# muellan/metacache

Measured on AMD Instinct MI355X. Metric: Mreads/min (150 bp), higher is better.
Workload: dtype u32

## Files before the change

metacache_amd/csrc/gw_kernels.hip:

```cpp
#include "device_common.h"

#include <algorithm>
#include <cstdlib>

namespace mcamd {

namespace {

constexpr uint32_t kGwNone = 0xFFFFFFFFu;
constexpr uint32_t kGwRounds = 128;
constexpr uint32_t kGwLoads = kGwRounds / 16;

struct __attribute__((packed, aligned(4))) U4 { uint32_t x, y, z, w; };

__device__ __forceinline__ uint32_t gw_block_shift(uint32_t maxWin)
{
    const uint32_t D = maxWin > 1 ? maxWin - 1 : 1;
    const uint32_t A = 32u - (uint32_t)__builtin_clz(64u * D - 1u);
    return A < 8u ? 8u : A;
}

template <uint32_t T1LOG2, uint32_t T2LOG2>
struct GwBloom {
    static constexpr uint32_t kW1 = (1u << T1LOG2) / 32, kW2 = (1u << T2LOG2) / 32, kWords = kW1 + kW2;
// ... 572 lines not shown
__device__ __forceinline__ uint32_t gw_count_numbers(const uint32_t (&v)[PER], uint2* slots, uint32_t* ck, const uint32_t lane)
{
    constexpr uint32_t kByteMask = ((1u << LOG2S) - 1u) << 3;
    char* base = reinterpret_cast<char*>(slots);
    auto key_at = [&](uint32_t off) -> uint32_t* { return reinterpret_cast<uint32_t*>(base + off); };
    uint32_t off[PER], old[PER];
    bool coll = false;
#pragma unroll
    for (uint32_t r = 0; r < PER; ++r) {
        off[r] = gw_slot<LOG2S>(v[r]);
        old[r] = v[r] != kGwNone ? atomicCAS(key_at(off[r]), kGwNone, v[r]) : v[r];
        coll = coll || (old[r] != kGwNone && old[r] != v[r]);
    }
    if (__ballot(coll)) {
#pragma unroll
        for (uint32_t r = 0; r < PER; ++r) {
            if (old[r] != kGwNone && old[r] != v[r]) {
                uint32_t o = off[r];
                for (;;) {
                    o = (o + 8u) & kByteMask;
                    old[r] = atomicCAS(key_at(o), kGwNone, v[r]);
                    if (old[r] == kGwNone || old[r] == v[r]) break;
                }
                off[r] = o;
            }
        }
    }
    uint32_t C = 0;
#pragma unroll
    for (uint32_t r = 0; r < PER; ++r) {
        if (v[r] != kGwNone) atomicAdd(key_at(off[r]) + 1, 1u);
        const bool claimed = v[r] != kGwNone && old[r] == kGwNone;
        const uint64_t m = __ballot(claimed);
        if (claimed) {
            const uint32_t at = __builtin_amdgcn_mbcnt_hi((uint32_t)(m >> 32), __builtin_amdgcn_mbcnt_lo((uint32_t)m, C));
            if (CKCAP == 0xFFFFFFFFu || at < CKCAP) ck[at] = off[r];
        }
        C += (uint32_t)__popcll(m);
    }
    return C;
}

template <uint32_t LOG2S, uint32_t PER, bool TAX>
__device__ __forceinline__ uint32_t gw_pick(const uint32_t* ck, const uint32_t C, uint2* slots, const uint32_t lane, const uint32_t maxWin,
                                            const uint32_t K, const uint32_t* __restrict__ taxkey, const DeviceTable& tab,
                                            uint32_t& owv, uint32_t& owh, uint32_t& owd)
{
    constexpr uint32_t kByteMask = ((1u << LOG2S) - 1u) << 3;
    const char* base = reinterpret_cast<const char*>(slots);
    uint32_t v[PER], R[PER];
#pragma unroll
    for (uint32_t r = 0; r < PER; ++r) {
        const uint2 c = r * 64 + lane < C ? *reinterpret_cast<const uint2*>(base + ck[r * 64 + lane]) : make_uint2(kGwNone, 0u);
        v[r] = c.x; R[r] = c.y;
    }
    uint32_t tgt[TAX ? PER : 1], thi[TAX ? PER : 1];
    if constexpr (TAX) {
#pragma unroll
        for (uint32_t r = 0; r < PER; ++r) tgt[r] = v[r] != kGwNone ? tab.gwDir[v[r] >> tab.gwDirShift] : 0u;
    }
    for (uint32_t d = 1; d < maxWin; ++d) {
        uint2 kc[PER]; uint32_t o[PER];
        bool chain = false;
#pragma unroll
        for (uint32_t r = 0; r < PER; ++r) {
            o[r] = gw_slot<LOG2S>(v[r] - d);
            kc[r] = *reinterpret_cast<const uint2*>(base + o[r]);
            if (v[r] == kGwNone) kc[r].x = kGwNone;
            chain = chain || (kc[r].x != v[r] - d && kc[r].x != kGwNone);
        }
        if (__ballot(chain)) {
#pragma unroll
            for (uint32_t r = 0; r < PER; ++r)
                while (kc[r].x != v[r] - d && kc[r].x != kGwNone) { o[r] = (o[r] + 8u) & kByteMask; kc[r] = *reinterpret_cast<const uint2*>(base + o[r]); }
        }
#pragma unroll
        for (uint32_t r = 0; r < PER; ++r)
            if (kc[r].x == v[r] - d) R[r] = ((R[r] & 0xFFFFu) + kc[r].y) | (d << 16);
    }
    uint32_t ptax[TAX ? PER : 1];
    if constexpr (TAX) {
#pragma unroll
        for (uint32_t r = 0; r < PER; ++r) {
            thi[r] = v[r] != kGwNone ? tab.gwBase[tgt[r] + 1] : 0u;
            while (v[r] != kGwNone && v[r] >= thi[r]) { ++tgt[r]; thi[r] = tab.gwBase[tgt[r] + 1]; }
            ptax[r] = v[r] != kGwNone ? taxkey[tgt[r]] : 0u;
        }
    }
    uint32_t live = 0;
#pragma unroll
    for (uint32_t r = 0; r < PER; ++r) {
        bool ok = v[r] != kGwNone;
        if constexpr (TAX) ok = ok && ptax[r] != 0;
        live |= ok ? (1u << r) : 0u;
    }
    uint32_t strong = 0;
    uint32_t wv = kGwNone, wh = 0, wd = 0;
    for (uint32_t rnd = 0; rnd < K; ++rnd) {
        uint32_t hh = 0, hv = kGwNone, hd = 0, hg = 0;
#pragma unroll
        for (uint32_t r = 0; r < PER; ++r) {
            const uint32_t h = R[r] & 0xFFFFu;
            const bool take = ((live >> r) & 1u) && (h > hh || (h == hh && v[r] < hv));
            if (take) { hh = h; hv = v[r]; hd = R[r] >> 16; if constexpr (TAX) hg = ptax[r]; }
        }
        const uint32_t mh = wave_max_u32(hh);
        if (mh == 0) break;
        const uint32_t mv = wave_min_u32(hh == mh ? hv : kGwNone);
        const uint32_t winner = __ffsll((unsigned long long)__ballot(hh == mh && hv == mv)) - 1;
        const uint32_t d = rdlane(hd, winner);
        if constexpr (TAX) {
            const uint32_t g = rdlane(hg, winner);
#pragma unroll
            for (uint32_t r = 0; r < PER; ++r) if (ptax[r] == g) live &= ~(1u << r);
        } else {
            const uint32_t from = mv - tab.gwGap, span = 2u * tab.gwGap;
#pragma unroll
            for (uint32_t r = 0; r < PER; ++r) if (v[r] - from <= span) live &= ~(1u << r);
        }
        if (lane == rnd) { wv = mv; wh = mh; wd = d; }
        strong += mh >= 2 ? 1u : 0u;
    }
    owv = wv; owh = wh; owd = wd;
    return strong;
}

template <bool TAX>
__device__ __forceinline__ bool gw_winners_out(const uint32_t lane, const uint32_t K, const uint32_t wv, const uint32_t wh, const uint32_t wd,
                                               const uint32_t wt, const uint32_t wlo, const uint32_t whi, mc_candidate_dev* __restrict__ out,
                                               uint32_t (&pickLo)[kLaneK], uint32_t (&pickHi)[kLaneK])
{
    bool again = false;
    if constexpr (!TAX) {
#pragma unroll
        for (uint32_t i = 0; i + 1 < kLaneK; ++i) {
            const uint32_t ti = rdlane(wt, i);
            again = again || (__ballot(lane > i && lane < K && wt == ti && ti != 0xFFFFFFFFu) != 0);
        }
    }
#pragma unroll
    for (uint32_t i = 0; i < kLaneK; ++i) { pickLo[i] = rdlane(wlo, i); pickHi[i] = rdlane(whi, i); }
    if (lane < K) {
        mc_candidate_dev e; e.tgt = wt; e.hits = wh; e.end = wv - wlo; e.beg = e.end - wd;
        if (wv == kGwNone) { e.tgt = 0xFFFFFFFFu; e.hits = 0; e.beg = 0; e.end = 0; }
        out[lane] = e;
    }
    return again;
}

}

namespace {

struct GwPend {
    bool pend = false;
    uint32_t q = 0, wv = kGwNone, wh = 0, wd = 0, dir = 0, b0 = 0, b1 = 0, b2 = 0;
    __device__ __forceinline__ void bases(const DeviceTable& tab)
    {
        if (pend && wv != kGwNone) { b0 = tab.gwBase[dir]; b1 = tab.gwBase[dir + 1]; b2 = tab.gwBase[min(dir + 2, tab.gwTargets)]; }
    }
    template <bool TAX>
    __device__ __forceinline__ void finish(const uint32_t lane, const uint32_t K, const DeviceTable& tab, const Workspace& ws, mc_candidate_dev* __restrict__ cands)
    {
        if (!pend) return;
        uint32_t t = 0xFFFFFFFFu, lo = 0, hi = 0;
        if (wv != kGwNone) {
            t = dir; lo = b0; hi = b1;
            if (wv >= b1) { ++t; lo = b1; hi = b2; }
            while (wv >= hi) { ++t; lo = hi; hi = tab.gwBase[t + 1]; }
        }
        uint32_t plo[kLaneK], phi[kLaneK];
        const bool again = gw_winners_out<TAX>(lane, K, wv, wh, wd, t, lo, hi, cands + (size_t)q * K, plo, phi);
        if (lane == 0) {
            if (again) { ws.hitScan[q] = ws.qstat[q].hits; ws.qflag[q] = kFlagCands; }
            else ws.qflag[q] = kFlagDone;
        }
        pend = false;
    }
};

template <uint32_t LOG2S, bool TAX, bool DEFER, bool LONG = false, class GetV, class EntF>
__device__ __forceinline__ bool gw_count_read(const uint32_t q, EntF&& entf, const uint32_t n2, const uint32_t maxWin, GetV&& getv,
                                              uint2* slots, uint32_t* ck, uint64_t* T, const uint32_t lane, const uint32_t grp, const uint32_t sub4,
                                              const uint32_t K, const uint32_t* __restrict__ taxkey, const DeviceTable& tab, const Workspace& ws,
                                              mc_candidate_dev* __restrict__ cands, GwPend& P)
{
    constexpr uint32_t kSlots = 1u << LOG2S, kList = kSlots / 2;
    {
        uint4* k4 = reinterpret_cast<uint4*>(slots);
#pragma unroll
        for (uint32_t i = 0; i < kSlots * 8 / 16 / 64; ++i) k4[i * 64 + lane] = make_uint4(kGwNone, 0u, kGwNone, 0u);
    }
    wave_lds_sync();
    uint32_t pickLo[kLaneK], pickHi[kLaneK];
#pragma unroll
    for (uint32_t i = 0; i < kLaneK; ++i) { pickLo[i] = 0; pickHi[i] = 0; }
    uint32_t strong = 0, wv = kGwNone, wh = 0, wd = 0;
    bool again = false;
    mc_candidate_dev* out = cands + (size_t)q * K;
    if constexpr (DEFER) P.bases(tab);
    uint32_t C = 0;
    auto body = [&](auto perc) {
        constexpr uint32_t PER = decltype(perc)::value;
        uint32_t v[PER];
#pragma unroll
        for (uint32_t r = 0; r < PER; ++r) v[r] = getv(r);
        C = gw_count_numbers<LOG2S, PER, LONG ? kList : 0xFFFFFFFFu>(v, slots, ck, lane);
    };
    const uint32_t per = (n2 + 63u) / 64u;
    if constexpr (LOG2S == 9) {
        if (per <= 1) body(std::integral_constant<uint32_t, 1>{});
        else if (per <= 2) body(std::integral_constant<uint32_t, 2>{});
        else if (per <= 3) body(std::integral_constant<uint32_t, 3>{});
        else if (!LONG || per <= 4) body(std::integral_constant<uint32_t, 4>{});
        else if constexpr (LONG) {
            if (per <= 6) body(std::integral_constant<uint32_t, 6>{});
            else body(std::integral_constant<uint32_t, 8>{});
        }
    } else if constexpr (LOG2S == 10) {
        if (per <= 6) body(std::integral_constant<uint32_t, 6>{});
        else body(std::integral_constant<uint32_t, 8>{});
    } else {
        if (per <= 10) body(std::integral_constant<uint32_t, 10>{});
        else if (per <= 12) body(std::integral_constant<uint32_t, 12>{});
        else body(std::integral_constant<uint32_t, kList / 64>{});
    }
    C = __builtin_amdgcn_readfirstlane(C);
    wave_lds_sync();
    if constexpr (LONG) {
        if (C > kList) {
            if constexpr (DEFER) P.template finish<TAX>(lane, K, tab, ws, cands);
            wave_lds_sync();
            return false;
        }
    }
    auto pick = [&](auto perc) {
        constexpr uint32_t PER = decltype(perc)::value;
        strong = gw_pick<LOG2S, PER, TAX>(ck, C, slots, lane, maxWin, K, taxkey, tab, wv, wh, wd);
    };
    if (C <= 64) pick(std::integral_constant<uint32_t, 1>{});
    else if (C <= 128) pick(std::integral_constant<uint32_t, 2>{});
    else if (C <= 256) pick(std::integral_constant<uint32_t, 4>{});
    else if constexpr (LOG2S >= 10) {
        if (C <= 512) pick(std::integral_constant<uint32_t, 8>{});
        else if constexpr (LOG2S >= 11) pick(std::integral_constant<uint32_t, 16>{});
    }
    strong = __builtin_amdgcn_readfirstlane(strong);
    if constexpr (DEFER) {
        P.template finish<TAX>(lane, K, tab, ws, cands);
        if (strong >= K) {
            P.pend = true; P.q = q; P.wv = wv; P.wh = wh; P.wd = wd;
            P.dir = wv != kGwNone ? tab.gwDir[wv >> tab.gwDirShift] : 0u;
            wave_lds_sync();
            return true;
        }
    }
    {
        uint32_t wt = 0xFFFFFFFFu, wlo = 0, whi = 0;
        if (wv != kGwNone) tab.gw_target_bounds(wv, wt, wlo, whi);
        again = gw_winners_out<TAX>(lane, K, wv, wh, wd, wt, wlo, whi, out, pickLo, pickHi);
    }
    bool done = true;
    if (again) {
        if (lane == 0) { ws.hitScan[q] = ws.qstat[q].hits; ws.qflag[q] = kFlagCands; }
        done = false;
    } else if (strong < K) {
        const uint2 r6 = entf();
        const uint32_t fbase = r6.x, nent = r6.y;
        if (TAX || nent > kBigEnt) {
            if (lane == 0) { ws.hitScan[q] = ws.qstat[q].hits; ws.qflag[q] = kFlagCands; }
            done = false;
        } else if constexpr (!TAX) {
            wave_lds_sync();
            const uint32_t sz = lane < nent ? (ws.psize[fbase + lane] & 0xFFFFu) : 0u;
            const uint64_t pay = lane < nent ? ws.ppay[fbase + lane] : 0ull;
            const uint32_t myR = sz > 1 ? (sz + 15u) >> 4 : 0u;
            const uint32_t incl = wave_incl_scan_u32(myR, lane), Rc = rdlane(incl, 63), start = incl - myR;
            uint32_t best[kLaneK];
#pragma unroll
            for (uint32_t i = 0; i < kLaneK; ++i) best[i] = kGwNone;
            uint32_t seen = 0;
            auto visit = [&](uint32_t g, bool valid) {
                if (!valid) return;
                bool skip = false;
#pragma unroll
                for (uint32_t i = 0; i < kLaneK; ++i) skip = skip || (i < strong && g - pickLo[i] < pickHi[i] - pickLo[i]);
                if (skip) return;
                ++seen;
                uint32_t c = g;
#pragma unroll
                for (uint32_t i = 0; i < kLaneK; ++i) { const uint32_t lo = min(best[i], c); c = max(best[i], c); best[i] = lo; }
            };
            visit(sz == 1 ? tab.gw_of(pay) : kGwNone, sz == 1);
            for (uint32_t r0 = 0; r0 < Rc; r0 += kGwRounds) {
                for (uint32_t i = lane; i < kGwRounds; i += 64) if (r0 + i >= Rc) T[i] = 0ull;
                const uint32_t jlo = r0 > start ? r0 - start : 0u, jhi = min(myR, r0 + kGwRounds > start ? r0 + kGwRounds - start : 0u);
                for (uint32_t j = jlo; j < jhi; ++j) T[start + j - r0] = (pay + 16ull * j) | ((uint64_t)min(16u, sz - 16u * j) << 40);
                wave_lds_sync();
#pragma unroll
                for (uint32_t u = 0; u < kGwLoads; ++u) {
                    const uint64_t rd = T[u * 16 + grp];
                    const int32_t rem = (int32_t)(uint32_t)(rd >> 40) - (int32_t)sub4;
                    if (rem > 0) {
                        const U4 t = *reinterpret_cast<const U4*>(tab.values32 + (rd & 0xFFFFFFFFFFull) + sub4);
                        visit(t.x, true); visit(t.y, rem > 1); visit(t.z, rem > 2); visit(t.w, rem > 3);
                    }
                }
                wave_lds_sync();
            }
            const bool dropped = seen > kLaneK;
            bool unsure = false;
            for (uint32_t rnd = strong; rnd < K; ++rnd) {
                if (__ballot(dropped && best[0] == kGwNone)) { unsure = true; break; }
                const uint32_t m = wave_min_u32(best[0]);
                mc_candidate_dev e; e.tgt = 0xFFFFFFFFu; e.hits = 0; e.beg = 0; e.end = 0;
                if (m != kGwNone) {
                    const uint32_t t = tab.gw_target(m), lo = tab.gwBase[t], hi = tab.gwBase[t + 1];
                    e.tgt = t; e.hits = 1; e.beg = e.end = m - lo;
                    uint32_t kept[kLaneK];
#pragma unroll
                    for (uint32_t i = 0; i < kLaneK; ++i) kept[i] = kGwNone;
                    uint32_t n = 0;
#pragma unroll
                    for (uint32_t i = 0; i < kLaneK; ++i) {
                        const bool stay = best[i] != kGwNone && !(best[i] - lo < hi - lo);
#pragma unroll
                        for (uint32_t j = 0; j < kLaneK; ++j) if (stay && j == n) kept[j] = best[i];
                        n += stay ? 1u : 0u;
                    }
#pragma unroll
                    for (uint32_t i = 0; i < kLaneK; ++i) best[i] = kept[i];
                }
                if (lane == 0) out[rnd] = e;
            }
            if (unsure) {
                if (lane == 0) { ws.hitScan[q] = ws.qstat[q].hits; ws.qflag[q] = kFlagCands; }
                done = false;
            }
        }
    }
    if (done && lane == 0) ws.qflag[q] = kFlagDone;
    wave_lds_sync();
    return true;
}

}

#ifndef MC_GW_COUNT_WPE
#define MC_GW_COUNT_WPE 6
#endif
template <uint32_t LOG2S, uint32_t WAVES, bool TAX>
__global__ __launch_bounds__(WAVES * 64, LOG2S == 9 ? MC_GW_COUNT_WPE : LOG2S == 10 ? 5 : 1) void gw_count_kernel(BatchView b, uint32_t s, DeviceTable tab, Workspace ws, uint32_t K,
                                                                                             const uint32_t* __restrict__ taxkey, mc_candidate_dev* __restrict__ cands,
                                                                                             uint32_t minN2)
{
    constexpr uint32_t kSlots = 1u << LOG2S, kList = kSlots / 2;
    static_assert(kGwRounds * 8 <= kSlots * 8, "step D's round table lives in the slot table, which is done with by then");
    __shared__ __attribute__((aligned(16))) uint2 slotS[WAVES][kSlots];
    __shared__ uint32_t ckS[WAVES][kList];
    const uint32_t lane = threadIdx.x & 63u, wave = __builtin_amdgcn_readfirstlane(threadIdx.x >> 6);
    uint2* slots = slotS[wave];
    uint32_t* ck = ckS[wave];
    uint64_t* T = reinterpret_cast<uint64_t*>(slotS[wave]);
    const uint32_t total = ws.midCount[kCntFilter];
    const uint4* __restrict__ work = ws.midList + list_at(kListFiltered, b.n);
    const uint4* __restrict__ work6 = ws.midList + list_at(kListFilter, b.n);
    const uint32_t nWaves = gridDim.x * WAVES;
    const uint32_t w0 = blockIdx.x * WAVES + wave;
    const uint32_t grp = lane >> 2, sub4 = (lane & 3u) * 4u;
    const uint32_t* __restrict__ pool = reinterpret_cast<const uint32_t*>(ws.bigPool);
    constexpr uint32_t kPre = LOG2S <= 10 ? kList / 64 : 1;
    uint32_t pre[kPre];
    auto fetch = [&](uint32_t off, uint32_t n) {
        if constexpr (LOG2S <= 10) {
#pragma unroll
            for (uint32_t r = 0; r < kPre; ++r) pre[r] = r * 64 + lane < n ? pool[off + r * 64 + lane] : kGwNone;
        }
    };
    constexpr bool kDefer = LOG2S <= 10;
    GwPend P;
    const uint32_t nmine = LOG2S == 9 ? total : ws.midCount[LOG2S == 10 ? kCnt512 : kCnt1024];
    const uint32_t kStep = LOG2S == 9 ? 64u : min(8u, max(1u, (nmine + nWaves - 1) / nWaves));
    const uint32_t* __restrict__ side = ws.sideList + list_at(LOG2S == 10 ? kSide512 : kSide1024, b.n);
    for (uint32_t chunk = w0 * kStep; chunk < nmine; chunk += nWaves * kStep) {
      const bool inb = lane < kStep && chunk + lane < nmine;
      const uint32_t myW = LOG2S == 9 ? chunk + lane : (inb ? side[chunk + lane] : 0u);
      const uint4 myRec = inb ? work[myW] : make_uint4(0, 0, kGwFallback, 0);
      uint64_t todo = __ballot(myRec.z <= kList && (minN2 == 0 || myRec.z > minN2) && myRec.w <= kHashWin);
      if (todo) { const uint32_t j = (uint32_t)__ffsll((unsigned long long)todo) - 1; fetch(rdlane(myRec.y, j), rdlane(myRec.z, j)); }
      while (todo) {
        const uint32_t j = (uint32_t)__ffsll((unsigned long long)todo) - 1;
        todo &= todo - 1;
        const uint32_t w = rdlane(myW, j), q = rdlane(myRec.x, j), n2 = rdlane(myRec.z, j), maxWin = rdlane(myRec.w, j);
        const uint32_t* __restrict__ src = pool + rdlane(myRec.y, j);
        uint32_t cur[kPre];
#pragma unroll
        for (uint32_t r = 0; r < kPre; ++r) cur[r] = pre[r];
        if (todo) { const uint32_t jn = (uint32_t)__ffsll((unsigned long long)todo) - 1; fetch(rdlane(myRec.y, jn), rdlane(myRec.z, jn)); }
        gw_count_read<LOG2S, TAX, kDefer>(q, [&]() -> uint2 { const uint4 r6 = work6[w]; return make_uint2(r6.y, r6.z & 0xFFFu); }, n2, maxWin, [&](uint32_t r) -> uint32_t {
            if constexpr (LOG2S <= 10) return cur[r < kPre ? r : 0];
            else return r * 64 + lane < n2 ? src[r * 64 + lane] : kGwNone;
        }, slots, ck, T, lane, grp, sub4, K, taxkey, tab, ws, cands, P);
      }
    }
    if constexpr (kDefer) { P.bases(tab); P.template finish<TAX>(lane, K, tab, ws, cands); }
}

constexpr uint32_t kGwCounted = 0x80000000u;

template <uint32_t WAVES, uint32_t TLOG2, bool TAX, uint32_t WPE = MC_GW_FILTER_WPE, bool LOOKUP = false>
__global__ __launch_bounds__(WAVES * 64, WPE) void gw_filter_count_kernel(BatchView b, DeviceTable tab, Workspace ws, uint32_t K, const uint32_t* __restrict__ taxkey,
                                                                                 mc_candidate_dev* __restrict__ cands, const uint32_t s)
{
    using Bloom = GwBloom<TLOG2, TLOG2>;
    constexpr uint32_t kKeep = WPE >= 6 ? 384 : 512;
    static_assert(kGwRounds * 8 >= 256 * 4, "the distinct numbers' slots take the place of the round table");
    constexpr bool kSeven = WPE >= 7;
    __shared__ __attribute__((aligned(16))) uint32_t bitS[WAVES][Bloom::kWords];
    __shared__ __attribute__((aligned(16))) uint64_t roundS[kSeven ? 1 : WAVES][kSeven ? 1 : kGwRounds];
    __shared__ __attribute__((aligned(16))) uint32_t keptS[WAVES][kKeep];
    const uint32_t lane = threadIdx.x & 63u, wave = __builtin_amdgcn_readfirstlane(threadIdx.x >> 6);
    uint32_t* bits = bitS[wave];
    uint64_t* T = kSeven ? reinterpret_cast<uint64_t*>(bits) : roundS[kSeven ? 0 : wave];
    uint32_t* kept = keptS[wave];
    const uint32_t total = LOOKUP ? b.n : ws.midCount[kCntFilter];
    uint4* const work = ws.midList + list_at(kListFilter, b.n);
    uint4* __restrict__ outRec = ws.midList + list_at(kListFiltered, b.n);
    const uint32_t nWaves = gridDim.x * WAVES;
    const uint32_t w0 = blockIdx.x * WAVES + wave;
    auto load_rec = [&](uint32_t w) -> uint4 { return (!LOOKUP && w < total) ? work[w] : make_uint4(0, 0, 0, 0); };
    const uint64_t sliceCap = ws.bigPoolCap / nWaves;
    uint32_t* const slice = reinterpret_cast<uint32_t*>(ws.bigPool) + (uint64_t)w0 * sliceCap;
    uint64_t sliceUsed = (LOOKUP && ws.sliceFill) ? ws.sliceFill[w0] : 0u;
    uint32_t deferred = 0;
    uint4 rec = load_rec(w0), recNext = load_rec(w0 + nWaves);
    uint32_t esz = 0; uint64_t epay = 0;
    auto load_entries = [&](const uint4& r) {
        if constexpr (LOOKUP) return;
        const uint32_t ne = (r.z >> 12) <= kGwSmallH ? min(r.z & 0xFFFu, 64u) : 0u;
        esz = lane < ne ? ws.psize[r.y + lane] : 0u;
        epay = lane < ne ? ws.ppay[r.y + lane] : 0ull;
    };
    load_entries(rec);
    constexpr uint32_t kLkSkip = 0xFFFFFFFFu;
    auto load_meta = [&](uint32_t q) -> uint2 {
        if (!LOOKUP || q >= b.n) return make_uint2(kLkSkip, 0u);
        const uint32_t o0 = ws.winOff[q], nf = (ws.winOff[q + 1] - o0) * s;
        return (ws.qflag[q] == kFlagProbe && nf <= 64u) ? make_uint2(o0 * s, nf) : make_uint2(kLkSkip, 0u);
    };
    auto load_feat = [&](const uint2& m) -> uint32_t { return (m.x != kLkSkip && lane < m.y) ? ws.features[m.x + lane] : 0xFFFFFFFFu; };
    uint2 m0 = load_meta(w0), m1 = load_meta(w0 + nWaves), m2 = load_meta(w0 + 2 * nWaves);
    uint32_t lkFeat = 0xFFFFFFFFu, lkNfeat = 0; uint64_t lkEnt = 0;
    if constexpr (LOOKUP) {
        const uint32_t f0 = load_feat(m0);
        lkFeat = load_feat(m1);
        lkNfeat = (uint32_t)__popcll(__ballot(f0 != 0xFFFFFFFFu));
        lkEnt = f0 != 0xFFFFFFFFu ? tab.direct[f0] : 0ull;
    }
    const uint32_t grp = lane >> 2, sub4 = (lane & 3u) * 4u;
    GwPend P;
    for (uint32_t w = w0; w < total; w += nWaves) {
        uint32_t q, nent, H, maxWin, sz, fbase = 0; uint64_t pay;
        uint32_t rix = 0xFFFFFFFFu;
        if constexpr (!LOOKUP) {
            q = rec.x; nent = rec.z & 0xFFFu; H = rec.z >> 12; maxWin = rec.w;
            sz = esz & 0xFFFFu; pay = epay;
            rec = recNext;
            recNext = load_rec(w + 2 * nWaves);
            load_entries(rec);
        } else {
            const uint2 cur = m0; const uint64_t e = lkEnt; const uint32_t nfeat = lkNfeat;
            lkNfeat = (uint32_t)__popcll(__ballot(lkFeat != 0xFFFFFFFFu));
            lkEnt = lkFeat != 0xFFFFFFFFu ? tab.direct[lkFeat] : 0ull;
            lkFeat = load_feat(m2);
            m0 = m1; m1 = m2; m2 = load_meta(w + 3 * nWaves);
            if (cur.x == kLkSkip) continue;
            q = w; fbase = cur.x;
            sz = (uint32_t)e & 0xFFFFu; pay = direct_payload(e);
            const uint64_t fm = __ballot(sz != 0u), sm = __ballot(sz == 1u);
            nent = (uint32_t)__popcll(fm);
            const uint32_t n1 = (uint32_t)__popcll(sm), lsz = sz > 1u ? sz : 0u;
            const uint32_t lincl = wave_incl_scan_u32(lsz, lane);
            H = n1 + rdlane(lincl, 63);
            maxWin = b.maxWin ? b.maxWin[q] : b.maxWinUniform;
            if (lane == 0) { QueryStat qs; qs.hits = H; qs.nfeat = nfeat; qs.nfound = nent; qs.nsteps = nfeat; ws.qstat[q] = qs; }
            if (H == 0) {
                if (lane < K) { mc_candidate_dev ev; ev.tgt = 0xFFFFFFFFu; ev.hits = 0; ev.beg = 0; ev.end = 0; cands[(size_t)q * K + lane] = ev; }
                if (lane == 0) { ws.hitScan[q] = 0u; ws.qflag[q] = kFlagDone; }
                continue;
            }
            {
                const uint32_t below = __builtin_amdgcn_mbcnt_hi((uint32_t)(fm >> 32), __builtin_amdgcn_mbcnt_lo((uint32_t)fm, 0u));
                const uint32_t sbelow = __builtin_amdgcn_mbcnt_hi((uint32_t)(sm >> 32), __builtin_amdgcn_mbcnt_lo((uint32_t)sm, 0u));
                if (sz != 0u) {
                    const uint32_t slot = sz == 1u ? sbelow : n1 + (below - sbelow);
                    const uint32_t off = sz == 1u ? slot : n1 + lincl - lsz;
                    ws.psize[fbase + slot] = sz | ((off & 0xFFFu) << 16);
                    ws.ppay[fbase + slot] = pay;
                } else if (lane < cur.y) ws.psize[fbase + nent + (lane - below)] = 0u;
            }
            const bool hashOK = nent <= kHashEnt && maxWin <= kHashWin;
            const bool bigOK = H > ws.bigMin && H > 64u && nent <= 0xFFFu && maxWin <= tab.gwGap && H <= kMaxHitsPerQuery;
            const uint32_t cls = bigOK ? kClassFilter : H <= 64 ? kListMid64 : H <= 128 ? (hashOK ? kListHash256 : kListMid128) : H <= kMidMax ? (hashOK ? kListHash256 : kListMid256)
                               : (H <= kHashMax && hashOK) ? (H <= kHashMax / 2 ? kListHash512 : kListHash1024) : kClassWave;
            if (lane == 0) {
                ws.hitScan[q] = (H <= kMaxHitsPerQuery && H > kLdsCap && !(cls >= kListHash512 && cls != kClassWave)) ? H : 0u;
                ws.qflag[q] = cls != kClassWave ? kFlagMid : kFlagCands;
                if (cls != kClassWave && cls != kClassFilter) {
                    const uint32_t at = atomicAdd(&ws.midCount[class_counter(cls)], 1u);
                    ws.midList[list_at(class_list(cls), b.n) + at] = make_uint4(q, fbase, nent | (H << 12), maxWin);
                }
            }
            if (cls != kClassFilter) continue;
        }
        auto slot_of = [&]() -> uint32_t {
            if constexpr (!LOOKUP) return w;
            else {
                if (rix == 0xFFFFFFFFu) {
                    uint32_t at = 0;
                    if (lane == 0) { at = atomicAdd(&ws.midCount[kCntFilter], 1u); work[at] = make_uint4(q, fbase, nent | (H << 12), maxWin); }
                    rix = rdlane(at, 0);
                }
                return rix;
            }
        };
        const uint32_t myR = sz > 1 ? (sz + 15u) >> 4 : 0u;
        const uint32_t incl = wave_incl_scan_u32(myR, lane), Rc = rdlane(incl, 63);
        if (H > kGwSmallH || nent > 64u || Rc > kGwRounds || maxWin > tab.gwGap || sliceCap - sliceUsed < kGwRounds * 16u + 64u) {
            const uint32_t at = slot_of();
            if (lane == 0) outRec[at] = make_uint4(q, 0u, kGwDefer, maxWin);
            ++deferred;
            continue;
        }
        auto clear_bits = [&]() {
            uint4* z4 = reinterpret_cast<uint4*>(bits);
#pragma unroll
            for (uint32_t i = 0; i < Bloom::kWords / 4 / 64; ++i) z4[i * 64 + lane] = make_uint4(0, 0, 0, 0);
        };
        if constexpr (!kSeven) clear_bits();
        gw_fill_rounds_scan(T, kept, lane, Rc, incl - myR, myR, sz, pay);
        wave_lds_sync();
        const GwFrame F(maxWin);
        const uint32_t nl = (Rc + 15u) >> 4;
        uint4 x[kGwLoads];
        gw_load_rounds(T, tab.values32, grp, sub4, x, nl);
        uint32_t rems = 0;
        if constexpr (kSeven) {
            rems = gw_pack_rems(T, grp, sub4, nl);
            wave_lds_sync();
            clear_bits();
            wave_lds_sync();
        }
        auto take_rounds = [&](auto check, GwSink& S) {
            constexpr bool CHECK = decltype(check)::value;
            if constexpr (kSeven) gw_take_rounds_packed<Bloom, CHECK>(bits, rems, F, S, x, nl);
            else gw_take_rounds<Bloom, CHECK>(bits, T, F, S, grp, sub4, x, nl);
        };
        const uint32_t sv = sz == 1 ? tab.gw_of(pay) : kGwNone;
        if (sv != kGwNone) Bloom::mark(bits, sv >> F.A);
        gw_mark_rounds<Bloom>(bits, x, F.A, nl);
        wave_lds_sync();
        const bool here = maxWin <= kHashWin;
        uint32_t n2;
        if (here) {
            GwSink S{kept, kKeep, 0u};
            gw_take<Bloom>(bits, F, S, sv, sv != kGwNone);
            take_rounds(std::true_type{}, S);
            n2 = S.n2;
        } else {
            GwSink S{slice + sliceUsed, (uint32_t)min((uint64_t)kGwMaxKept, sliceCap - sliceUsed), 0u};
            gw_take<Bloom>(bits, F, S, sv, sv != kGwNone);
            take_rounds(std::false_type{}, S);
            n2 = S.n2;
        }
        if (here && n2 <= kKeep) {
            if constexpr (!LOOKUP) { if (lane == 0) outRec[w] = make_uint4(q, 0u, kGwCounted | n2, maxWin); }
            wave_lds_sync();
            const bool counted = gw_count_read<9, TAX, true, true>(q, [&]() -> uint2 {
                                            if constexpr (LOOKUP) { wave_mem_sync(); return make_uint2(fbase, nent); }
                                            else { const uint4 r6 = work[w]; return make_uint2(r6.y, r6.z & 0xFFFu); }
                                        }, n2, maxWin,
                                        [&](uint32_t r) -> uint32_t { return r * 64 + lane < n2 ? kept[r * 64 + lane] : kGwNone; },
                                        reinterpret_cast<uint2*>(bits), kSeven ? kept : reinterpret_cast<uint32_t*>(T), kSeven ? reinterpret_cast<uint64_t*>(kept) : T,
                                        lane, grp, sub4, K, taxkey, tab, ws, cands, P);
            if (!counted && kSeven) {
                const uint32_t at = slot_of();
                if (lane == 0) outRec[at] = make_uint4(q, 0u, kGwDefer, maxWin);
                ++deferred;
                wave_lds_sync();
            } else if (!counted) {
#pragma unroll
                for (uint32_t r = 0; r < kKeep / 64; ++r) if (r * 64 + lane < n2) slice[sliceUsed + r * 64 + lane] = kept[r * 64 + lane];
                const uint32_t at = slot_of();
                if (lane == 0) outRec[at] = make_uint4(q, (uint32_t)((uint64_t)w0 * sliceCap + sliceUsed), n2, maxWin);
                sliceUsed += n2;
                wave_lds_sync();
            }
            continue;
        }
        if (here) {
            GwSink S{slice + sliceUsed, (uint32_t)min((uint64_t)kGwMaxKept, sliceCap - sliceUsed), 0u};
            gw_take<Bloom>(bits, F, S, sv, sv != kGwNone);
            take_rounds(std::false_type{}, S);
            n2 = S.n2;
        }
        const uint32_t room = (uint32_t)min((uint64_t)kGwMaxKept, sliceCap - sliceUsed);
        const bool fallback = n2 > room;
        const uint32_t at = slot_of();
        if (lane == 0) {
            if (fallback) { ws.hitScan[q] = H; ws.qflag[q] = kFlagCands; outRec[at] = make_uint4(q, 0u, kGwFallback, maxWin); }
            else outRec[at] = make_uint4(q, (uint32_t)((uint64_t)w0 * sliceCap + sliceUsed), n2, maxWin);
        }
        if (!fallback) sliceUsed += n2;
        wave_lds_sync();
    }
    P.bases(tab); P.template finish<TAX>(lane, K, tab, ws, cands);
    if (lane == 0) {
        if (ws.sliceFill) ws.sliceFill[w0] = (uint32_t)sliceUsed;
        if (deferred) atomicAdd(&ws.midCount[kCntSecond], deferred);
    }
}

constexpr uint32_t kGwBigSorted = 8192;

template <bool TAX>
__device__ __forceinline__ void gw_sorted_scan(const uint32_t* __restrict__ g, const uint32_t first, const uint32_t end, const uint32_t D,
                                               const DeviceTable& tab, const uint32_t* __restrict__ taxkey, const uint32_t K, uint32_t* ring,
                                               const uint32_t lane, LaneCand (&top)[kLaneK], uint32_t (&toptax)[kLaneK])
{
    uint32_t cT = 0xFFFFFFFFu, cHits = 0, cBeg = 0, cEnd = 0, cLo = 0, cHi = 0;
    uint32_t lowFst = 0;
    uint32_t gnext = first + lane < end ? g[first + lane] : 0xFFFFFFFFu;
    uint32_t dnext = gnext != 0xFFFFFFFFu ? tab.gwDir[gnext >> tab.gwDirShift] : 0u;
    for (uint32_t base = first; base < end; base += 64) {
        const uint32_t cnt = min(64u, end - base), ei = base + lane;
        const bool valid = lane < cnt;
        const uint32_t gi = gnext, di = dnext;
        gnext = ei + 64u < end ? g[ei + 64u] : 0xFFFFFFFFu;
        ring[ei & 127u] = gi;
        wave_lds_sync();
        const uint32_t want = gi - D;
        const uint32_t rlo = base >= first + 64u ? base - 64u : first;
        uint32_t lo = 0, hi = 0;
        bool glob = false;
        if (valid) {
            if (lowFst >= rlo) { lo = lowFst; hi = ei; }
            else if (ring[rlo & 127u] < want) { lo = rlo + 1u; hi = ei; }
            else { lo = lowFst; hi = rlo; glob = true; }
        }
        while (__ballot(!glob && lo < hi)) {
            const uint32_t mid = (lo + hi) >> 1;
            if (!glob && lo < hi) { if (ring[mid & 127u] < want) lo = mid + 1u; else hi = mid; }
        }
        while (__ballot(glob && lo < hi)) {
            const uint32_t mid = (lo + hi) >> 1;
            if (glob && lo < hi) { if (g[mid] < want) lo = mid + 1u; else hi = mid; }
        }
        const uint32_t fst = lo;
        const uint32_t gf = !valid ? 0u : fst >= rlo ? ring[fst & 127u] : g[fst];
        lowFst = rdlane(fst, cnt - 1u);
        uint32_t t = 0xFFFFFFFFu, tlo = 0, thi = 0;
        const bool inCur = cT != 0xFFFFFFFFu && (gi - cLo) < (cHi - cLo);
        if (valid) {
            if (inCur) { t = cT; tlo = cLo; thi = cHi; }
            else {
                t = di;
                const uint32_t b0 = tab.gwBase[t], b1 = tab.gwBase[t + 1], b2 = tab.gwBase[min(t + 2, tab.gwTargets)];
                tlo = b0; thi = b1;
                if (gi >= b1) { ++t; tlo = b1; thi = b2; }
                while (gi >= thi) { ++t; tlo = thi; thi = tab.gwBase[t + 1]; }
            }
        }
        if (cT != 0xFFFFFFFFu && rdlane(t, 0) != cT && lane == 0) {
            LaneCand c; c.tgt = cT; c.hits = cHits; c.beg = cBeg; c.end = cEnd;
            top_insert(top, toptax, c, K, TAX ? taxkey : nullptr, 0xFFFFFFFFu);
        }
        uint32_t val = valid ? (((ei - fst + 1u) << 6) | (63u - lane)) : 0u;
#pragma unroll
        for (uint32_t d = 1; d < 64; d <<= 1) {
            const uint32_t ov = (uint32_t)__shfl_up((int)val, d), ot = (uint32_t)__shfl_up((int)t, d);
            if (lane >= d && ot == t) val = max(val, ov);
        }
        const uint32_t tnext = (uint32_t)__shfl_down((int)t, 1);
        const bool tail = valid && (lane + 1u >= cnt || tnext != t);
        const uint32_t wl = 63u - (val & 63u);
        LaneCand c; c.tgt = t; c.hits = val >> 6;
        c.beg = (uint32_t)__shfl((int)gf, (int)wl) - tlo; c.end = (uint32_t)__shfl((int)gi, (int)wl) - tlo;
        if (t == cT && cHits >= c.hits) { c.hits = cHits; c.beg = cBeg; c.end = cEnd; }
        const bool last = base + 64u >= end;
        if (tail && (last || lane + 1u < cnt)) top_insert(top, toptax, c, K, TAX ? taxkey : nullptr, 0xFFFFFFFFu);
        cT = rdlane(c.tgt, cnt - 1u); cHits = rdlane(c.hits, cnt - 1u); cBeg = rdlane(c.beg, cnt - 1u); cEnd = rdlane(c.end, cnt - 1u);
        cLo = rdlane(tlo, cnt - 1u); cHi = rdlane(thi, cnt - 1u);
        dnext = gnext != 0xFFFFFFFFu ? tab.gwDir[gnext >> tab.gwDirShift] : 0u;
    }
    wave_lds_sync();
}

template <bool TAX, class Put>
__device__ __forceinline__ uint32_t gw_sorted_rounds(LaneCand (&top)[kLaneK], uint32_t (&toptax)[kLaneK], const uint32_t K, Put&& put)
{
    uint32_t strong = 0;
    for (uint32_t rnd = 0; rnd < K; ++rnd) {
        const uint32_t mh = wave_max_u32(top[0].hits);
        mc_candidate_dev ev; ev.tgt = 0xFFFFFFFFu; ev.hits = 0; ev.beg = 0; ev.end = 0;
        uint32_t mtax = 0;
        if (mh != 0) {
            const uint32_t mt = wave_min_u32(top[0].hits == mh ? top[0].tgt : 0xFFFFFFFFu);
            const uint32_t me = wave_min_u32(top[0].hits == mh && top[0].tgt == mt ? top[0].end : 0xFFFFFFFFu);
            const uint32_t winner = __ffsll((unsigned long long)__ballot(top[0].hits == mh && top[0].tgt == mt && top[0].end == me)) - 1;
            ev.tgt = mt; ev.hits = mh; ev.end = me; ev.beg = rdlane(top[0].beg, winner);
            mtax = rdlane(toptax[0], winner);
            strong += mh >= 2 ? 1u : 0u;
            LaneCand kept[kLaneK]; uint32_t ktax[kLaneK];
#pragma unroll
            for (uint32_t i = 0; i < kLaneK; ++i) { kept[i].tgt = 0xFFFFFFFFu; kept[i].hits = 0; kept[i].beg = 0; kept[i].end = 0; ktax[i] = 0; }
            uint32_t nk = 0;
#pragma unroll
            for (uint32_t i = 0; i < kLaneK; ++i) {
                const bool stay = top[i].hits != 0 && (TAX ? toptax[i] != mtax : top[i].tgt != mt);
#pragma unroll
                for (uint32_t jj = 0; jj < kLaneK; ++jj) if (stay && jj == nk) { kept[jj] = top[i]; ktax[jj] = toptax[i]; }
                nk += stay ? 1u : 0u;
            }
#pragma unroll
            for (uint32_t i = 0; i < kLaneK; ++i) { top[i] = kept[i]; toptax[i] = ktax[i]; }
        }
        put(rnd, ev, mtax);
    }
    return strong;
}

constexpr uint32_t kGwFewBig = 1024;
template <bool TAX, bool BIG>
__global__ __launch_bounds__(BIG ? 1024 : 256) void gw_sorted_cands_kernel(BatchView b, DeviceTable tab, Workspace ws, uint32_t K, const uint32_t* __restrict__ taxkey,
                                                                           mc_candidate_dev* __restrict__ cands)
{
    constexpr uint32_t kWaves = BIG ? 16u : 4u;
    __shared__ uint32_t ringS[kWaves][128];
    __shared__ mc_candidate_dev pickS[kWaves][kLaneK];
    __shared__ uint32_t ptaxS[kWaves][kLaneK];
    const uint32_t lane = threadIdx.x & 63u, wave = __builtin_amdgcn_readfirstlane(threadIdx.x >> 6);
    uint32_t* ring = ringS[wave];
    const uint4* __restrict__ work = ws.midList + list_at(kListFiltered, b.n);
    const uint32_t* __restrict__ side = ws.sideList + list_at(kSideSorted, b.n);
    auto finish = [&](uint32_t q, uint32_t strong) {
        if (lane == 0) {
            if (strong < K) { ws.hitScan[q] = ws.qstat[q].hits; ws.qflag[q] = kFlagCands; }
            else ws.qflag[q] = kFlagDone;
        }
    };
    if constexpr (!BIG) {
        const uint32_t nWaves = gridDim.x * 4, w0 = blockIdx.x * 4 + wave;
        const uint32_t nmine = ws.midCount[kCntSorted];
        uint32_t lo = 0, hi = nmine;
        while (lo < hi) { const uint32_t mid = (lo + hi) >> 1; if (work[side[mid]].z > kGwBigSorted) lo = mid + 1u; else hi = mid; }
        const uint32_t nbig = min(lo, kGwFewBig);
        if (w0 == 0 && lane == 0) ws.midCount[kCntSortedBig] = nbig;
        for (uint32_t i = nbig + w0; i < nmine; i += nWaves) {
            const uint32_t w = side[i];
            const uint4 rec = work[w];
            const uint32_t q = rec.x, n = rec.z, maxWin = rec.w;
            LaneCand top[kLaneK];
            uint32_t toptax[kLaneK];
#pragma unroll
            for (uint32_t j = 0; j < kLaneK; ++j) { top[j].tgt = 0xFFFFFFFFu; top[j].hits = 0; top[j].beg = 0; top[j].end = 0; toptax[j] = 0; }
            gw_sorted_scan<TAX>(ws.bigPool2 + rec.y, 0u, n, maxWin - 1u, tab, taxkey, K, ring, lane, top, toptax);
            mc_candidate_dev* out = cands + (size_t)q * K;
            const uint32_t strong = gw_sorted_rounds<TAX>(top, toptax, K, [&](uint32_t rnd, const mc_candidate_dev& ev, uint32_t) { if (lane == 0) out[rnd] = ev; });
            finish(q, strong);
// ... 109 lines not shown
```

Before: 20470.

## Defer per-query entry stores to paths that actually consume them

In the lookup-fused path, the psize/ppay compacted entry arrays were previously written for every query before classification. Now they are written only when a query leaves the fast path (non-filter class, deferral, fallback, or needing candidate rescans). Queries fully resolved in-wave skip the writes, and when needed the entries are recomputed by reloading features and direct-table values. This trades global stores for occasional redundant reloads and recomputation on slow paths.

```diff
diff --git a/metacache_amd/csrc/gw_kernels.hip b/metacache_amd/csrc/gw_kernels.hip
--- a/metacache_amd/csrc/gw_kernels.hip
+++ b/metacache_amd/csrc/gw_kernels.hip
@@ -748,6 +748,59 @@
 
 namespace {
 
+__device__ __forceinline__ void lk_store_entries(const Workspace& ws, const uint32_t fbase, const uint32_t nf, const uint32_t lane, const uint32_t sz, const uint64_t pay,
+                                                 const uint64_t fm, const uint64_t sm, const uint32_t lincl)
+{
+    const uint32_t nent = (uint32_t)__popcll(fm), n1 = (uint32_t)__popcll(sm), lsz = sz > 1u ? sz : 0u;
+    const uint32_t below = __builtin_amdgcn_mbcnt_hi((uint32_t)(fm >> 32), __builtin_amdgcn_mbcnt_lo((uint32_t)fm, 0u));
+    const uint32_t sbelow = __builtin_amdgcn_mbcnt_hi((uint32_t)(sm >> 32), __builtin_amdgcn_mbcnt_lo((uint32_t)sm, 0u));
+    if (sz != 0u) {
+        const uint32_t slot = sz == 1u ? sbelow : n1 + (below - sbelow);
+        const uint32_t off = sz == 1u ? slot : n1 + lincl - lsz;
+        ws.psize[fbase + slot] = sz | ((off & 0xFFFu) << 16);
+        ws.ppay[fbase + slot] = pay;
+    } else if (lane < nf) ws.psize[fbase + nent + (lane - below)] = 0u;
+}
+__device__ __forceinline__ void lk_store_entries(const Workspace& ws, const uint32_t fbase, const uint32_t nf, const uint32_t lane, const uint32_t sz, const uint64_t pay)
+{
+    lk_store_entries(ws, fbase, nf, lane, sz, pay, __ballot(sz != 0u), __ballot(sz == 1u), wave_incl_scan_u32(sz > 1u ? sz : 0u, lane));
+}
+__device__ __forceinline__ void lk_load_entries(const Workspace& ws, const DeviceTable& tab, const uint32_t s, const uint32_t q, const uint32_t lane,
+                                                uint32_t& fbase, uint32_t& nf, uint32_t& sz, uint64_t& pay)
+{
+    const uint32_t o0 = ws.winOff[q];
+    fbase = o0 * s; nf = (ws.winOff[q + 1] - o0) * s;
+    const uint32_t f = lane < nf ? ws.features[fbase + lane] : 0xFFFFFFFFu;
+    const uint64_t e = f != 0xFFFFFFFFu ? tab.direct[f] : 0ull;
+    sz = (uint32_t)e & 0xFFFFu; pay = direct_payload(e);
+}
+
+struct GwEntRecord {
+    const uint4* rec;
+    __device__ __forceinline__ uint2 where() const { const uint4 r6 = *rec; return make_uint2(r6.y, r6.z & 0xFFFu); }
+    __device__ __forceinline__ void load(const Workspace& ws, const DeviceTable&, uint32_t, uint32_t fbase, uint32_t nent, uint32_t lane, uint32_t& sz, uint64_t& pay) const
+    {
+        sz = lane < nent ? (ws.psize[fbase + lane] & 0xFFFFu) : 0u;
+        pay = lane < nent ? ws.ppay[fbase + lane] : 0ull;
+    }
+    __device__ __forceinline__ void leave(const Workspace&, const DeviceTable&, uint32_t, uint32_t) const {}
+};
+struct GwEntLookup {
+    uint32_t fbase, nent, s;
+    __device__ __forceinline__ uint2 where() const { return make_uint2(fbase, nent); }
+    __device__ __forceinline__ void load(const Workspace& ws, const DeviceTable& tab, uint32_t q, uint32_t, uint32_t, uint32_t lane, uint32_t& sz, uint64_t& pay) const
+    {
+        uint32_t fb, nf;
+        lk_load_entries(ws, tab, s, q, lane, fb, nf, sz, pay);
+    }
+    __device__ __forceinline__ void leave(const Workspace& ws, const DeviceTable& tab, uint32_t q, uint32_t lane) const
+    {
+        uint32_t fb, nf, sz; uint64_t pay;
+        lk_load_entries(ws, tab, s, q, lane, fb, nf, sz, pay);
+        lk_store_entries(ws, fb, nf, lane, sz, pay);
+    }
+};
+
 struct GwPend {
     bool pend = false;
     uint32_t q = 0, wv = kGwNone, wh = 0, wd = 0, dir = 0, b0 = 0, b1 = 0, b2 = 0;
@@ -755,8 +808,8 @@
     {
         if (pend && wv != kGwNone) { b0 = tab.gwBase[dir]; b1 = tab.gwBase[dir + 1]; b2 = tab.gwBase[min(dir + 2, tab.gwTargets)]; }
     }
-    template <bool TAX>
-    __device__ __forceinline__ void finish(const uint32_t lane, const uint32_t K, const DeviceTable& tab, const Workspace& ws, mc_candidate_dev* __restrict__ cands)
+    template <bool TAX, class Ent>
+    __device__ __forceinline__ void finish(const uint32_t lane, const uint32_t K, const DeviceTable& tab, const Workspace& ws, mc_candidate_dev* __restrict__ cands, const Ent& ent)
     {
         if (!pend) return;
         uint32_t t = 0xFFFFFFFFu, lo = 0, hi = 0;
@@ -767,6 +820,7 @@
         }
         uint32_t plo[kLaneK], phi[kLaneK];
         const bool again = gw_winners_out<TAX>(lane, K, wv, wh, wd, t, lo, hi, cands + (size_t)q * K, plo, phi);
+        if (again) ent.leave(ws, tab, q, lane);
         if (lane == 0) {
             if (again) { ws.hitScan[q] = ws.qstat[q].hits; ws.qflag[q] = kFlagCands; }
             else ws.qflag[q] = kFlagDone;
@@ -775,8 +829,8 @@
     }
 };
 
-template <uint32_t LOG2S, bool TAX, bool DEFER, bool LONG = false, class GetV, class EntF>
-__device__ __forceinline__ bool gw_count_read(const uint32_t q, EntF&& entf, const uint32_t n2, const uint32_t maxWin, GetV&& getv,
+template <uint32_t LOG2S, bool TAX, bool DEFER, bool LONG = false, class GetV, class Ent>
+__device__ __forceinline__ bool gw_count_read(const uint32_t q, const Ent& ent, const uint32_t n2, const uint32_t maxWin, GetV&& getv,
                                               uint2* slots, uint32_t* ck, uint64_t* T, const uint32_t lane, const uint32_t grp, const uint32_t sub4,
                                               const uint32_t K, const uint32_t* __restrict__ taxkey, const DeviceTable& tab, const Workspace& ws,
                                               mc_candidate_dev* __restrict__ cands, GwPend& P)
@@ -825,7 +879,7 @@
     wave_lds_sync();
     if constexpr (LONG) {
         if (C > kList) {
-            if constexpr (DEFER) P.template finish<TAX>(lane, K, tab, ws, cands);
+            if constexpr (DEFER) P.template finish<TAX>(lane, K, tab, ws, cands, ent);
             wave_lds_sync();
             return false;
         }
@@ -843,7 +897,7 @@
     }
     strong = __builtin_amdgcn_readfirstlane(strong);
     if constexpr (DEFER) {
-        P.template finish<TAX>(lane, K, tab, ws, cands);
+        P.template finish<TAX>(lane, K, tab, ws, cands, ent);
         if (strong >= K) {
             P.pend = true; P.q = q; P.wv = wv; P.wh = wh; P.wd = wd;
             P.dir = wv != kGwNone ? tab.gwDir[wv >> tab.gwDirShift] : 0u;
@@ -858,18 +912,20 @@
     }
     bool done = true;
     if (again) {
+        ent.leave(ws, tab, q, lane);
         if (lane == 0) { ws.hitScan[q] = ws.qstat[q].hits; ws.qflag[q] = kFlagCands; }
         done = false;
     } else if (strong < K) {
-        const uint2 r6 = entf();
+        const uint2 r6 = ent.where();
         const uint32_t fbase = r6.x, nent = r6.y;
         if (TAX || nent > kBigEnt) {
+            ent.leave(ws, tab, q, lane);
             if (lane == 0) { ws.hitScan[q] = ws.qstat[q].hits; ws.qflag[q] = kFlagCands; }
             done = false;
         } else if constexpr (!TAX) {
             wave_lds_sync();
-            const uint32_t sz = lane < nent ? (ws.psize[fbase + lane] & 0xFFFFu) : 0u;
-            const uint64_t pay = lane < nent ? ws.ppay[fbase + lane] : 0ull;
+            uint32_t sz; uint64_t pay;
+            ent.load(ws, tab, q, fbase, nent, lane, sz, pay);
             const uint32_t myR = sz > 1 ? (sz + 15u) >> 4 : 0u;
             const uint32_t incl = wave_incl_scan_u32(myR, lane), Rc = rdlane(incl, 63), start = incl - myR;
             uint32_t best[kLaneK];
@@ -930,6 +986,7 @@
                 if (lane == 0) out[rnd] = e;
             }
             if (unsure) {
+                ent.leave(ws, tab, q, lane);
                 if (lane == 0) { ws.hitScan[q] = ws.qstat[q].hits; ws.qflag[q] = kFlagCands; }
                 done = false;
             }
@@ -993,13 +1050,13 @@
 #pragma unroll
         for (uint32_t r = 0; r < kPre; ++r) cur[r] = pre[r];
         if (todo) { const uint32_t jn = (uint32_t)__ffsll((unsigned long long)todo) - 1; fetch(rdlane(myRec.y, jn), rdlane(myRec.z, jn)); }
-        gw_count_read<LOG2S, TAX, kDefer>(q, [&]() -> uint2 { const uint4 r6 = work6[w]; return make_uint2(r6.y, r6.z & 0xFFFu); }, n2, maxWin, [&](uint32_t r) -> uint32_t {
+        gw_count_read<LOG2S, TAX, kDefer>(q, GwEntRecord{work6 + w}, n2, maxWin, [&](uint32_t r) -> uint32_t {
             if constexpr (LOG2S <= 10) return cur[r < kPre ? r : 0];
             else return r * 64 + lane < n2 ? src[r * 64 + lane] : kGwNone;
         }, slots, ck, T, lane, grp, sub4, K, taxkey, tab, ws, cands, P);
       }
     }
-    if constexpr (kDefer) { P.bases(tab); P.template finish<TAX>(lane, K, tab, ws, cands); }
+    if constexpr (kDefer) { P.bases(tab); P.template finish<TAX>(lane, K, tab, ws, cands, GwEntRecord{work6}); }
 }
 
 constexpr uint32_t kGwCounted = 0x80000000u;
@@ -1056,7 +1113,7 @@
     const uint32_t grp = lane >> 2, sub4 = (lane & 3u) * 4u;
     GwPend P;
     for (uint32_t w = w0; w < total; w += nWaves) {
-        uint32_t q, nent, H, maxWin, sz, fbase = 0; uint64_t pay;
+        uint32_t q, nent, H, maxWin, sz, fbase = 0, nfs = 0; uint64_t pay;
         uint32_t rix = 0xFFFFFFFFu;
         if constexpr (!LOOKUP) {
             q = rec.x; nent = rec.z & 0xFFFu; H = rec.z >> 12; maxWin = rec.w;
@@ -1071,7 +1128,7 @@
             lkFeat = load_feat(m2);
             m0 = m1; m1 = m2; m2 = load_meta(w + 3 * nWaves);
             if (cur.x == kLkSkip) continue;
-            q = w; fbase = cur.x;
+            q = w; fbase = cur.x; nfs = cur.y;
             sz = (uint32_t)e & 0xFFFFu; pay = direct_payload(e);
             const uint64_t fm = __ballot(sz != 0u), sm = __ballot(sz == 1u);
             nent = (uint32_t)__popcll(fm);
@@ -1085,16 +1142,6 @@
                 if (lane == 0) { ws.hitScan[q] = 0u; ws.qflag[q] = kFlagDone; }
                 continue;
             }
-            {
-                const uint32_t below = __builtin_amdgcn_mbcnt_hi((uint32_t)(fm >> 32), __builtin_amdgcn_mbcnt_lo((uint32_t)fm, 0u));
-                const uint32_t sbelow = __builtin_amdgcn_mbcnt_hi((uint32_t)(sm >> 32), __builtin_amdgcn_mbcnt_lo((uint32_t)sm, 0u));
-                if (sz != 0u) {
-                    const uint32_t slot = sz == 1u ? sbelow : n1 + (below - sbelow);
-                    const uint32_t off = sz == 1u ? slot : n1 + lincl - lsz;
-                    ws.psize[fbase + slot] = sz | ((off & 0xFFFu) << 16);
-                    ws.ppay[fbase + slot] = pay;
-                } else if (lane < cur.y) ws.psize[fbase + nent + (lane - below)] = 0u;
-            }
             const bool hashOK = nent <= kHashEnt && maxWin <= kHashWin;
             const bool bigOK = H > ws.bigMin && H > 64u && nent <= 0xFFFu && maxWin <= tab.gwGap && H <= kMaxHitsPerQuery;
             const uint32_t cls = bigOK ? kClassFilter : H <= 64 ? kListMid64 : H <= 128 ? (hashOK ? kListHash256 : kListMid128) : H <= kMidMax ? (hashOK ? kListHash256 : kListMid256)
@@ -1107,8 +1154,9 @@
                     ws.midList[list_at(class_list(cls), b.n) + at] = make_uint4(q, fbase, nent | (H << 12), maxWin);
                 }
             }
-            if (cls != kClassFilter) continue;
-        }
+            if (cls != kClassFilter) { lk_store_entries(ws, fbase, nfs, lane, sz, pay, fm, sm, lincl); continue; }
+        }
+        auto entries_out = [&]() { if constexpr (LOOKUP) GwEntLookup{fbase, nent, s}.leave(ws, tab, q, lane); };
         auto slot_of = [&]() -> uint32_t {
             if constexpr (!LOOKUP) return w;
             else {
@@ -1123,6 +1171,7 @@
         const uint32_t myR = sz > 1 ? (sz + 15u) >> 4 : 0u;
         const uint32_t incl = wave_incl_scan_u32(myR, lane), Rc = rdlane(incl, 63);
         if (H > kGwSmallH || nent > 64u || Rc > kGwRounds || maxWin > tab.gwGap || sliceCap - sliceUsed < kGwRounds * 16u + 64u) {
+            if constexpr (LOOKUP) lk_store_entries(ws, fbase, nfs, lane, sz, pay);
             const uint32_t at = slot_of();
             if (lane == 0) outRec[at] = make_uint4(q, 0u, kGwDefer, maxWin);
             ++deferred;
@@ -1172,14 +1221,17 @@
         if (here && n2 <= kKeep) {
             if constexpr (!LOOKUP) { if (lane == 0) outRec[w] = make_uint4(q, 0u, kGwCounted | n2, maxWin); }
             wave_lds_sync();
-            const bool counted = gw_count_read<9, TAX, true, true>(q, [&]() -> uint2 {
-                                            if constexpr (LOOKUP) { wave_mem_sync(); return make_uint2(fbase, nent); }
-                                            else { const uint4 r6 = work[w]; return make_uint2(r6.y, r6.z & 0xFFFu); }
-                                        }, n2, maxWin,
+            auto count = [&](const auto& ent) {
+                return gw_count_read<9, TAX, true, true>(q, ent, n2, maxWin,
                                         [&](uint32_t r) -> uint32_t { return r * 64 + lane < n2 ? kept[r * 64 + lane] : kGwNone; },
                                         reinterpret_cast<uint2*>(bits), kSeven ? kept : reinterpret_cast<uint32_t*>(T), kSeven ? reinterpret_cast<uint64_t*>(kept) : T,
                                         lane, grp, sub4, K, taxkey, tab, ws, cands, P);
+            };
+            bool counted;
+            if constexpr (LOOKUP) counted = count(GwEntLookup{fbase, nent, s});
+            else counted = count(GwEntRecord{work + w});
             if (!counted && kSeven) {
+                entries_out();
                 const uint32_t at = slot_of();
                 if (lane == 0) outRec[at] = make_uint4(q, 0u, kGwDefer, maxWin);
                 ++deferred;
@@ -1187,6 +1239,7 @@
             } else if (!counted) {
 #pragma unroll
                 for (uint32_t r = 0; r < kKeep / 64; ++r) if (r * 64 + lane < n2) slice[sliceUsed + r * 64 + lane] = kept[r * 64 + lane];
+                entries_out();
                 const uint32_t at = slot_of();
                 if (lane == 0) outRec[at] = make_uint4(q, (uint32_t)((uint64_t)w0 * sliceCap + sliceUsed), n2, maxWin);
                 sliceUsed += n2;
@@ -1202,6 +1255,7 @@
         }
         const uint32_t room = (uint32_t)min((uint64_t)kGwMaxKept, sliceCap - sliceUsed);
         const bool fallback = n2 > room;
+        entries_out();
         const uint32_t at = slot_of();
         if (lane == 0) {
             if (fallback) { ws.hitScan[q] = H; ws.qflag[q] = kFlagCands; outRec[at] = make_uint4(q, 0u, kGwFallback, maxWin); }
@@ -1210,7 +1264,9 @@
         if (!fallback) sliceUsed += n2;
         wave_lds_sync();
     }
-    P.bases(tab); P.template finish<TAX>(lane, K, tab, ws, cands);
+    P.bases(tab);
+    if constexpr (LOOKUP) P.template finish<TAX>(lane, K, tab, ws, cands, GwEntLookup{0u, 0u, s});
+    else P.template finish<TAX>(lane, K, tab, ws, cands, GwEntRecord{work});
     if (lane == 0) {
         if (ws.sliceFill) ws.sliceFill[w0] = (uint32_t)sliceUsed;
         if (deferred) atomicAdd(&ws.midCount[kCntSecond], deferred);
```

Result: faster. 20840, median of 6 (+1.8%).
